# IN2-ViAUn/Exploration-of-Potential

Measured on AMD Instinct MI355X. Metric: training images/sec, YOLOX-l 24p 640x640 bf16, higher is better.
Workload: dtype bf16; 1 GPU; YOLOX-l-24p (CSPDarknet53+PAFPN+24p head) train step, 640x640, batch 20/GPU, 10 GTs/img, SimOTA + 24-circle GIoU loss, SGD nesterov; global_batch=20, parallelism=dp1, hip_graph=forward and backward as two lanes of captured segments, loss, update

## Files before the change

### exploration-of-potential_amd/csrc/elementwise.hip

```cpp
#include <stdio.h>
#include <stdlib.h>
#include "common.h"

namespace {

constexpr int MAX_BLOCKS = 2048;

__device__ __forceinline__ void load8(const bf16* p, float (&v)[8]) {
    bf16x8 t = *reinterpret_cast<const bf16x8*>(p);
#pragma unroll
    for (int i = 0; i < 8; ++i) v[i] = (float)t[i];
}
__device__ __forceinline__ void store8(bf16* p, const float (&v)[8]) {
    bf16x8 t;
#pragma unroll
    for (int i = 0; i < 8; ++i) t[i] = (bf16)v[i];
    *reinterpret_cast<bf16x8*>(p) = t;
}

struct RowMap {
    int tpr, rpb;
    __device__ RowMap(int C, int nt = 256) { tpr = C >> 3; rpb = tpr >= nt ? 1 : nt / tpr; }
};

template <int ACT, bool RES>
__global__ __launch_bounds__(256) void bn_act_fwd_kernel(const bf16* z, long ld_z, const long long* stats, int reps,
                                                         const float* gamma, const float* beta, float* rmean,
                                                         float* rvar, long* nbt, long* nbt2, float* save, bf16* y, long ld_y,
                                                         const bf16* res_, long ld_res, long M, int C, float eps,
                                                         float momentum) {
    constexpr int act = ACT;
    const bf16* res = RES ? res_ : nullptr;
    extern __shared__ float lds[];
    const int CP = C + (C >> 3);
    float* sc = lds;
    float* sh = lds + CP;
    auto pad = [](int c) { return c + (c >> 3); };
    for (int c = threadIdx.x; c < C; c += 256) {
        long long i1 = 0, i2 = 0;
        const float gmm = gamma[c], bta = beta[c];
        for (int rb = 0; rb < reps; rb += 8) {
            long long a[8], b[8];
#pragma unroll
            for (int r = 0; r < 8; ++r) {
                const int rr = rb + r < reps ? rb + r : rb;
                a[r] = stats[(long)rr * 2 * C + c];
                b[r] = stats[(long)rr * 2 * C + C + c];
            }
#pragma unroll
            for (int r = 0; r < 8; ++r) {
                i1 += rb + r < reps ? a[r] : 0ll;
                i2 += rb + r < reps ? b[r] : 0ll;
            }
        }
        const float mean = from_fix(i1) / (float)M;
        float var = from_fix(i2) / (float)M - mean * mean;
        var = var < 0.f ? 0.f : var;
        const float invstd = rsqrtf(var + eps);
        const float s_ = gmm * invstd;
        sc[pad(c)] = s_;
        sh[pad(c)] = bta - mean * s_;
        if (blockIdx.x == 0) {
            save[c] = mean;
            save[C + c] = invstd;
            if (rmean) {
                const float unb = M > 1 ? var * (float)M / (float)(M - 1) : var;
                rmean[c] = (1.f - momentum) * rmean[c] + momentum * mean;
                rvar[c] = (1.f - momentum) * rvar[c] + momentum * unb;
            }
        }
    }
    if (blockIdx.x == 0 && threadIdx.x == 0) {
        if (nbt) *nbt += 1;
        if (nbt2) *nbt2 += 1;
    }
    __syncthreads();
    const int cgs = C >> 3;
    const long total = M * cgs;
    const long stride = (long)gridDim.x * 256;
    constexpr int U = 4;
    const bool fixed_group = stride % cgs == 0;
    const int g_fixed = (int)(((long)blockIdx.x * 256 + threadIdx.x) % cgs);
    float rsc[8], rsh[8];
#pragma unroll
    for (int j = 0; j < 8; ++j) { rsc[j] = sc[g_fixed * 9 + j]; rsh[j] = sh[g_fixed * 9 + j]; }
    const long m_fixed = ((long)blockIdx.x * 256 + threadIdx.x) / cgs, m_step = stride / cgs;
    int it = 0;
    for (long i = (long)blockIdx.x * 256 + threadIdx.x; i < total; i += U * stride, ++it) {
        long mm[U];
        int gg[U];
        bf16x8 v[U], r[U];
#pragma unroll
        for (int k = 0; k < U; ++k) {
            const long ik = i + k * stride;
            const bool ok = ik < total;
            if (fixed_group) {
                mm[k] = ok ? m_fixed + (long)(it * U + k) * m_step : -1;
                gg[k] = g_fixed;
            } else {
                mm[k] = ok ? ik / cgs : -1;
                gg[k] = ok ? (int)(ik - mm[k] * cgs) : 0;
            }
            if (ok) {
                v[k] = *reinterpret_cast<const bf16x8*>(z + mm[k] * ld_z + gg[k] * 8);
                if constexpr (RES) r[k] = *reinterpret_cast<const bf16x8*>(res + mm[k] * ld_res + gg[k] * 8);
            }
        }
#pragma unroll
        for (int k = 0; k < U; ++k) {
            if (mm[k] < 0) break;
            bf16x8 o;
#pragma unroll
            for (int j = 0; j < 8; ++j) {
                const float a_ = fixed_group ? rsc[j] : sc[gg[k] * 9 + j];
                const float b_ = fixed_group ? rsh[j] : sh[gg[k] * 9 + j];
                const float u = fmaf((float)v[k][j], a_, b_);
                if constexpr (RES) o[j] = (bf16)(act_fwd(u, act) + (float)r[k][j]);
                else o[j] = (bf16)act_fwd(u, act);
            }
            *reinterpret_cast<bf16x8*>(y + mm[k] * ld_y + gg[k] * 8) = o;
        }
    }
}


template <int UNROLL, int NT, int ACT>
__device__ __forceinline__ void bn_bwd_reduce_body(const bf16* dy, long ld_dy, const bf16* z, long ld_z,
                                                   const float* save, const float* gamma,
                                                   const float* beta, long long* dgamma, long long* dbeta,
                                                   long M, int C, int reps, const int bid, const int nblk) {
    constexpr int act = ACT;
    __shared__ float red[NT][8 + 1];
    const RowMap rm(C, NT);
    const int tid = threadIdx.x;
    for (int cg0 = 0; cg0 < (C >> 3); cg0 += NT) {
        const int cg = cg0 + tid % rm.tpr;
        const int slot = rm.tpr >= NT ? 0 : tid / rm.tpr;
        const bool active = slot < rm.rpb && cg < (C >> 3);
        float sg[8] = {0, 0, 0, 0, 0, 0, 0, 0}, sb[8] = {0, 0, 0, 0, 0, 0, 0, 0};
        if (active) {
            const long step = (long)nblk * rm.rpb;
            const long m_first = (long)bid * rm.rpb + slot;
            bf16x8 vdy[UNROLL], vz[UNROLL];
#pragma unroll
            for (int k = 0; k < UNROLL; ++k) {
                const long mm = m_first + k * step < M ? m_first + k * step : (m_first < M ? m_first : 0);
                vdy[k] = *reinterpret_cast<const bf16x8*>(dy + mm * ld_dy + cg * 8);
                vz[k] = *reinterpret_cast<const bf16x8*>(z + mm * ld_z + cg * 8);
            }
            __builtin_amdgcn_sched_barrier(0);
            float sc[8], sh[8], iv[8], mi[8];
#pragma unroll
            for (int j = 0; j < 8; ++j) {
                const int c = cg * 8 + j;
                const float mean = save[c], inv = save[C + c];
                sc[j] = gamma[c] * inv; sh[j] = beta[c] - mean * sc[j]; iv[j] = inv; mi[j] = mean * inv;
            }
            for (long m = m_first; m < M; m += UNROLL * step) {
#pragma unroll
                for (int k = 0; k < UNROLL; ++k) {
                    if (m + k * step >= M) break;
#pragma unroll
                    for (int j = 0; j < 8; ++j) {
                        const float zz = (float)vz[k][j];
                        const float du = (float)vdy[k][j] * act_grad(fmaf(zz, sc[j], sh[j]), act);
                        sb[j] += du;
                        sg[j] = fmaf(du, fmaf(zz, iv[j], -mi[j]), sg[j]);
                    }
                }
                if (m + UNROLL * step < M) {
#pragma unroll
                    for (int k = 0; k < UNROLL; ++k) {
                        const long mn = m + (UNROLL + k) * step;
                        const long mm = mn < M ? mn : m;
                        vdy[k] = *reinterpret_cast<const bf16x8*>(dy + mm * ld_dy + cg * 8);
                        vz[k] = *reinterpret_cast<const bf16x8*>(z + mm * ld_z + cg * 8);
                    }
                }
            }
        }
        const int ngrp = min(min(rm.tpr, NT), (C >> 3) - cg0);
#pragma unroll
        for (int half = 0; half < 2; ++half) {
#pragma unroll
            for (int j = 0; j < 8; ++j) red[tid][j] = half ? sb[j] : sg[j];
            __syncthreads();
            for (int t = tid; t < ngrp * 8; t += NT) {
                const int g = t >> 3, v = t & 7;
                float a = 0.f;
                for (int sl = 0; sl < rm.rpb; ++sl) a += red[sl * rm.tpr + g][v];
                long long* dst = (half ? dbeta : dgamma) + (long)(bid % reps) * 2 * C + (cg0 + g) * 8 + v;
                atomicAdd((unsigned long long*)dst, (unsigned long long)to_fix_g(a));
            }
            __syncthreads();
        }
    }
}

template <int UNROLL, int NT, int ACT>
__global__ __launch_bounds__(NT) void bn_act_bwd_reduce_kernel(const bf16* dy, long ld_dy, const bf16* z, long ld_z,
                                                               const float* save, const float* gamma,
                                                               const float* beta, long long* dgamma, long long* dbeta,
                                                               long M, int C, int reps) {
    bn_bwd_reduce_body<UNROLL, NT, ACT>(dy, ld_dy, z, ld_z, save, gamma, beta, dgamma, dbeta, M, C, reps, (int)blockIdx.x, (int)gridDim.x);
}

template <int UNROLL, int ACT, bool ACC, bool COH>
__device__ __forceinline__ void bn_bwd_apply_body(const bf16* dy, long ld_dy, const bf16* z, long ld_z,
                                                  const float* save, const float* gamma, const float* beta,
                                                  const long long* dgamma, const long long* dbeta, float* ggrad,
                                                  float* bgrad, bf16* dz, long ld_dz, long M, int C, int reps, const int bid, const int nblk) {
    constexpr int act = ACT;
    const RowMap rm(C);
    const int tid = threadIdx.x;
    const float invM = 1.f / (float)M;
    extern __shared__ float folded[];
    for (int i = tid; i < 2 * C; i += 256) {
        const long long* src = i < C ? dgamma + i : dbeta + (i - C);
        long long acc = 0;
        bool bad = false;
        for (int rb = 0; rb < reps; rb += 8) {
            long long a[8];
#pragma unroll
            for (int r = 0; r < 8; ++r) {
                const long long* q = src + (long)(rb + r < reps ? rb + r : rb) * 2 * C;
                a[r] = COH ? __hip_atomic_load(q, __ATOMIC_RELAXED, __HIP_MEMORY_SCOPE_AGENT) : *q;
            }
#pragma unroll
            for (int r = 0; r < 8; ++r) {
                acc += rb + r < reps ? a[r] : 0ll;
                bad = bad || fixg_bad(a[r]);
            }
        }
        folded[i] = bad ? __builtin_nanf("") : from_fix_g(acc);
    }
    __syncthreads();
    for (int cg = tid % rm.tpr; cg < (C >> 3); cg += 256) {
        const int slot = rm.tpr >= 256 ? 0 : tid / rm.tpr;
        if (slot >= rm.rpb) break;
        float sc[8], sh[8], k1[8], k2[8], k3[8];
        float cm[8], ci[8], cg_[8], cb[8], csg[8], csb[8];
        {
            const f32x4* pm = reinterpret_cast<const f32x4*>(save + cg * 8);
            const f32x4* pi = reinterpret_cast<const f32x4*>(save + C + cg * 8);
            const f32x4* pg = reinterpret_cast<const f32x4*>(gamma + cg * 8);
            const f32x4* pb = reinterpret_cast<const f32x4*>(beta + cg * 8);
            const f32x4 m0 = pm[0], m1 = pm[1], i0 = pi[0], i1 = pi[1], g0 = pg[0], g1 = pg[1], b0 = pb[0], b1 = pb[1];
            const f32x4 s0 = *reinterpret_cast<const f32x4*>(folded + cg * 8), s1 = *reinterpret_cast<const f32x4*>(folded + cg * 8 + 4);
            const f32x4 t0 = *reinterpret_cast<const f32x4*>(folded + C + cg * 8), t1 = *reinterpret_cast<const f32x4*>(folded + C + cg * 8 + 4);
#pragma unroll
            for (int j = 0; j < 4; ++j) {
                cm[j] = m0[j]; cm[4 + j] = m1[j]; ci[j] = i0[j]; ci[4 + j] = i1[j]; cg_[j] = g0[j]; cg_[4 + j] = g1[j]; cb[j] = b0[j]; cb[4 + j] = b1[j];
                csg[j] = s0[j]; csg[4 + j] = s1[j]; csb[j] = t0[j]; csb[4 + j] = t1[j];
            }
        }
#pragma unroll
        for (int j = 0; j < 8; ++j) {
            const float mean = cm[j], inv = ci[j], g = cg_[j];
            const float sg_ = csg[j], sb_ = csb[j];
            sc[j] = g * inv; sh[j] = cb[j] - mean * sc[j];
            k1[j] = g * inv;
            k3[j] = k1[j] * inv * (sg_ * invM);
            k2[j] = k1[j] * (sb_ * invM) - k3[j] * mean;
        }
        if (bid == 0 && slot == 0 && ggrad) {
            f32x4* pgg = reinterpret_cast<f32x4*>(ggrad + cg * 8);
            f32x4* pbg = reinterpret_cast<f32x4*>(bgrad + cg * 8);
            f32x4 a0 = pgg[0], a1 = pgg[1], c0 = pbg[0], c1 = pbg[1];
#pragma unroll
            for (int j = 0; j < 4; ++j) {
                a0[j] += csg[j]; a1[j] += csg[4 + j];
                c0[j] += csb[j]; c1[j] += csb[4 + j];
            }
            pgg[0] = a0; pgg[1] = a1; pbg[0] = c0; pbg[1] = c1;
        }
        const long step = (long)nblk * rm.rpb;
        for (long m = (long)bid * rm.rpb + slot; m < M; m += UNROLL * step) {
            bf16x8 vdy[UNROLL], vz[UNROLL];
#pragma unroll
            for (int k = 0; k < UNROLL; ++k) {
                const long mm = m + k * step;
                if (mm < M) {
                    vdy[k] = __builtin_nontemporal_load(reinterpret_cast<const bf16x8*>(dy + mm * ld_dy + cg * 8));
                    vz[k] = __builtin_nontemporal_load(reinterpret_cast<const bf16x8*>(z + mm * ld_z + cg * 8));
                }
            }
#pragma unroll
            for (int k = 0; k < UNROLL; ++k) {
                const long mm = m + k * step;
                if (mm >= M) break;
                bf16x8 o;
#pragma unroll
                for (int j = 0; j < 8; ++j) {
                    const float zz = (float)vz[k][j];
                    const float du = (float)vdy[k][j] * act_grad(fmaf(zz, sc[j], sh[j]), act);
                    o[j] = (bf16)fmaf(-k3[j], zz, fmaf(k1[j], du, -k2[j]));
                }
                if (ACC) {
                    const bf16x8 old = *reinterpret_cast<const bf16x8*>(dz + mm * ld_dz + cg * 8);
#pragma unroll
                    for (int j = 0; j < 8; ++j) o[j] = (bf16)((float)old[j] + (float)o[j]);
                }
                *reinterpret_cast<bf16x8*>(dz + mm * ld_dz + cg * 8) = o;
            }
        }
    }
}

template <int UNROLL, int ACT, bool ACC = false>
__global__ __launch_bounds__(256) void bn_act_bwd_apply_kernel(const bf16* dy, long ld_dy, const bf16* z, long ld_z,
                                                               const float* save, const float* gamma, const float* beta,
                                                               const long long* dgamma, const long long* dbeta, float* ggrad,
                                                               float* bgrad, bf16* dz, long ld_dz, long M, int C, int reps) {
    bn_bwd_apply_body<UNROLL, ACT, ACC, false>(dy, ld_dy, z, ld_z, save, gamma, beta, dgamma, dbeta, ggrad, bgrad, dz, ld_dz, M, C, reps,
                                               (int)blockIdx.x, (int)gridDim.x);
}

__device__ unsigned g_bn_barrier_timeouts;

template <int ACT>
__global__ __launch_bounds__(256) void bn_act_bwd_fused_kernel(const bf16* dy, long ld_dy, const bf16* z, long ld_z,
                                                               const float* save, const float* gamma, const float* beta,
                                                               long long* dgamma, long long* dbeta, float* ggrad, float* bgrad,
                                                               bf16* dz, long ld_dz, long M, int C, int reps, unsigned* bar) {
    const int bid = (int)blockIdx.x, nblk = (int)gridDim.x;
    bn_bwd_reduce_body<4, 256, ACT>(dy, ld_dy, z, ld_z, save, gamma, beta, dgamma, dbeta, M, C, reps, bid, nblk);
    __syncthreads();
    if (threadIdx.x == 0) {
        __threadfence();
        __hip_atomic_fetch_add(bar, 1u, __ATOMIC_RELEASE, __HIP_MEMORY_SCOPE_AGENT);
        int tries = 0;
        while (__hip_atomic_load(bar, __ATOMIC_ACQUIRE, __HIP_MEMORY_SCOPE_AGENT) < (unsigned)nblk) {
            __builtin_amdgcn_s_sleep(2);
            if (++tries > (1 << 16)) { atomicAdd(&g_bn_barrier_timeouts, 1u); break; }
        }
    }
    __syncthreads();
    bn_bwd_apply_body<4, ACT, false, true>(dy, ld_dy, z, ld_z, save, gamma, beta, dgamma, dbeta, ggrad, bgrad, dz, ld_dz, M, C, reps, bid, nblk);
}

int flat_grid(long M, int C, int per_thread) {
    long blocks = (M * (C >> 3) + 256L * per_thread - 1) / (256L * per_thread);
    return (int)(blocks < 1 ? 1 : (blocks > MAX_BLOCKS ? MAX_BLOCKS : blocks));
}
int rows_grid(long M, int C, int rows_per_thread, int max_blocks, int nt = 256) {
    int tpr = C >> 3;
    int rpb = tpr >= nt ? 1 : nt / tpr;
    long blocks = (M + (long)rpb * rows_per_thread - 1) / ((long)rpb * rows_per_thread);
    return (int)(blocks < 1 ? 1 : (blocks > max_blocks ? max_blocks : blocks));
}

__global__ __launch_bounds__(256) void stem_pack_kernel(const float* img, bf16* rows, int B, int IH, int IW, int ld) {
    constexpr int TP = 32;
    __shared__ __attribute__((aligned(16))) bf16 tile[TP][120];
    const int FH = IH >> 1, FW = IW >> 1;
    const long npix = (long)B * FH * FW;
    const int chunks = ld >> 3;
    for (long p0 = (long)blockIdx.x * TP; p0 < npix; p0 += (long)gridDim.x * TP) {
        for (int it = threadIdx.x; it < 9 * TP; it += 256) {
            const int tap = it / TP, lp = it - tap * TP;
            const long pix = p0 + lp;
            float v[12] = {0.f, 0.f, 0.f, 0.f, 0.f, 0.f, 0.f, 0.f, 0.f, 0.f, 0.f, 0.f};
            if (pix < npix) {
                const int n = (int)(pix / ((long)FH * FW));
                const int rem = (int)(pix - (long)n * FH * FW);
                const int oy = rem / FW, ox = rem - oy * FW;
                const int fy = oy + tap / 3 - 1, fx = ox + tap % 3 - 1;
                if (fy >= 0 && fy < FH && fx >= 0 && fx < FW) {
#pragma unroll
                    for (int ch = 0; ch < 3; ++ch)
#pragma unroll
                        for (int yp = 0; yp < 2; ++yp) {
                            const float2 t = *reinterpret_cast<const float2*>(img + (((long)n * 3 + ch) * IH + 2 * fy + yp) * IW + 2 * fx);
                            v[(0 * 2 + yp) * 3 + ch] = t.x;
                            v[(1 * 2 + yp) * 3 + ch] = t.y;
                        }
                }
            }
#pragma unroll
            for (int j = 0; j < 12; ++j) tile[lp][tap * 12 + j] = (bf16)v[j];
        }
        if (threadIdx.x < TP) {
#pragma unroll
            for (int j = 108; j < 120; ++j) tile[threadIdx.x][j] = (bf16)0.f;
        }
        __syncthreads();
        for (int it = threadIdx.x; it < TP * chunks; it += 256) {
            const int lp = it / chunks, c = it - lp * chunks;
            const long pix = p0 + lp;
            if (pix >= npix) continue;
            bf16x8 o = {0, 0, 0, 0, 0, 0, 0, 0};
            if (c * 8 < 120) o = *reinterpret_cast<const bf16x8*>(&tile[lp][c * 8]);
            *reinterpret_cast<bf16x8*>(rows + pix * ld + c * 8) = o;
        }
        __syncthreads();
    }
}

__global__ __launch_bounds__(256) void focus_pack_kernel(const float* img, bf16* out, int B, int IH, int IW) {
    const int FH = IH >> 1, FW = IW >> 1;
    const long npix = (long)B * FH * FW;
    for (long pix = (long)blockIdx.x * 256 + threadIdx.x; pix < npix; pix += (long)gridDim.x * 256) {
        const int n = (int)(pix / ((long)FH * FW));
        const int rem = (int)(pix - (long)n * FH * FW);
        const int fy = rem / FW, fx = rem - fy * FW;
        float v[12];
#pragma unroll
        for (int ch = 0; ch < 3; ++ch)
#pragma unroll
            for (int yp = 0; yp < 2; ++yp) {
                const float2 t = *reinterpret_cast<const float2*>(img + (((long)n * 3 + ch) * IH + 2 * fy + yp) * IW + 2 * fx);
                v[(0 * 2 + yp) * 3 + ch] = t.x;
                v[(1 * 2 + yp) * 3 + ch] = t.y;
            }
        bf16x8 lo, hi = {0, 0, 0, 0, 0, 0, 0, 0};
#pragma unroll
        for (int j = 0; j < 8; ++j) lo[j] = (bf16)v[j];
#pragma unroll
        for (int j = 8; j < 12; ++j) hi[j - 8] = (bf16)v[j];
        *reinterpret_cast<bf16x8*>(out + pix * 16) = lo;
        *reinterpret_cast<bf16x8*>(out + pix * 16 + 8) = hi;
    }
}

__global__ __launch_bounds__(256) void spp_fwd_kernel(const bf16* x, long ld_x, bf16* y5, bf16* y9, bf16* y13, long ld_y,
                                                      uint8_t* idx, int B, int H, int W, int C) {
    const int cgs = C >> 3;
    const long total = (long)B * H * W * cgs;
    const long plane = (long)B * H * W * C;
    for (long i = (long)blockIdx.x * 256 + threadIdx.x; i < total; i += (long)gridDim.x * 256) {
        const int cg = (int)(i % cgs);
        const long pix = i / cgs;
        const int n = (int)(pix / (H * W));
        const int rem = (int)(pix - (long)n * H * W);
        const int py = rem / W, px = rem - py * W;
        float m5[8], m9[8], m13[8];
        uint8_t i5[8], i9[8], i13[8];
#pragma unroll
        for (int j = 0; j < 8; ++j) { m5[j] = m9[j] = m13[j] = -INFINITY; i5[j] = i9[j] = i13[j] = 0x88; }
        for (int dy = -6; dy <= 6; ++dy) {
            const int yy = py + dy;
            if (yy < 0 || yy >= H) continue;
            for (int dx = -6; dx <= 6; ++dx) {
                const int xx = px + dx;
                if (xx < 0 || xx >= W) continue;
                float v[8];
                load8(x + ((long)(n * H + yy) * W + xx) * ld_x + cg * 8, v);
                const uint8_t code = (uint8_t)(((dy + 8) << 4) | (dx + 8));
                const bool in9 = dy >= -4 && dy <= 4 && dx >= -4 && dx <= 4;
                const bool in5 = dy >= -2 && dy <= 2 && dx >= -2 && dx <= 2;
#pragma unroll
                for (int j = 0; j < 8; ++j) {
                    if (v[j] > m13[j] || v[j] != v[j]) { m13[j] = v[j]; i13[j] = code; }
                    if (in9 && (v[j] > m9[j] || v[j] != v[j])) { m9[j] = v[j]; i9[j] = code; }
                    if (in5 && (v[j] > m5[j] || v[j] != v[j])) { m5[j] = v[j]; i5[j] = code; }
                }
            }
        }
        store8(y5 + pix * ld_y + cg * 8, m5);
        store8(y9 + pix * ld_y + cg * 8, m9);
        store8(y13 + pix * ld_y + cg * 8, m13);
        uint8_t* ip = idx + pix * C + cg * 8;
#pragma unroll
        for (int j = 0; j < 8; ++j) { ip[j] = i5[j]; ip[plane + j] = i9[j]; ip[2 * plane + j] = i13[j]; }
    }
}

__global__ __launch_bounds__(256) void spp_row_kernel(const bf16* x, long ld_x, bf16* h, uint8_t* hx, int B, int H, int W, int C) {
    const int cgs = C >> 3;
    const long total = (long)B * H * W * cgs;
    const long plane = (long)B * H * W * C;
    for (long i = (long)blockIdx.x * 256 + threadIdx.x; i < total; i += (long)gridDim.x * 256) {
        const int cg = (int)(i % cgs);
        const long pix = i / cgs;
        const int px = (int)(pix % W);
        float m5[8], m9[8], m13[8];
        uint8_t i5[8], i9[8], i13[8];
#pragma unroll
        for (int j = 0; j < 8; ++j) { m5[j] = m9[j] = m13[j] = -INFINITY; i5[j] = i9[j] = i13[j] = 8; }
#pragma unroll
        for (int dx = -6; dx <= 6; ++dx) {
            const int xx = px + dx;
            if (xx < 0 || xx >= W) continue;
            float v[8];
            load8(x + (pix + dx) * ld_x + cg * 8, v);
            const uint8_t code = (uint8_t)(dx + 8);
            const bool in9 = dx >= -4 && dx <= 4, in5 = dx >= -2 && dx <= 2;
#pragma unroll
            for (int j = 0; j < 8; ++j) {
                if (v[j] > m13[j] || v[j] != v[j]) { m13[j] = v[j]; i13[j] = code; }
                if (in9 && (v[j] > m9[j] || v[j] != v[j])) { m9[j] = v[j]; i9[j] = code; }
                if (in5 && (v[j] > m5[j] || v[j] != v[j])) { m5[j] = v[j]; i5[j] = code; }
            }
        }
        bf16* hp = h + pix * C + cg * 8;
        store8(hp, m5); store8(hp + plane, m9); store8(hp + 2 * plane, m13);
        uint8_t* ip = hx + pix * C + cg * 8;
#pragma unroll
        for (int j = 0; j < 8; ++j) { ip[j] = i5[j]; ip[plane + j] = i9[j]; ip[2 * plane + j] = i13[j]; }
    }
}

__global__ __launch_bounds__(256) void spp_col_kernel(const bf16* h, const uint8_t* hx, bf16* y5, bf16* y9, bf16* y13, long ld_y,
                                                      uint8_t* idx, int B, int H, int W, int C) {
    const int cgs = C >> 3;
    const long total = (long)B * H * W * cgs;
    const long plane = (long)B * H * W * C;
    for (long i = (long)blockIdx.x * 256 + threadIdx.x; i < total; i += (long)gridDim.x * 256) {
        const int cg = (int)(i % cgs);
        const long pix = i / cgs;
        const int py = (int)((pix / W) % H);
        float m[3][8];
        uint8_t id[3][8];
#pragma unroll
        for (int w = 0; w < 3; ++w)
#pragma unroll
            for (int j = 0; j < 8; ++j) { m[w][j] = -INFINITY; id[w][j] = 0x88; }
#pragma unroll
        for (int dy = -6; dy <= 6; ++dy) {
            const int yy = py + dy;
            if (yy < 0 || yy >= H) continue;
            const long q = (pix + (long)dy * W) * C + cg * 8;
#pragma unroll
            for (int w = 0; w < 3; ++w) {
                const int r = 2 + 2 * w;
                if (dy < -r || dy > r) continue;
                float v[8];
                load8(h + w * plane + q, v);
                const uint2 cx = *reinterpret_cast<const uint2*>(hx + w * plane + q);
#pragma unroll
                for (int j = 0; j < 8; ++j) {
                    const unsigned c = ((j < 4 ? cx.x : cx.y) >> (8 * (j & 3))) & 0xFF;
                    if (v[j] > m[w][j] || v[j] != v[j]) { m[w][j] = v[j]; id[w][j] = (uint8_t)(((dy + 8) << 4) | c); }
                }
            }
        }
        store8(y5 + pix * ld_y + cg * 8, m[0]);
        store8(y9 + pix * ld_y + cg * 8, m[1]);
        store8(y13 + pix * ld_y + cg * 8, m[2]);
        uint8_t* ip = idx + pix * C + cg * 8;
#pragma unroll
        for (int j = 0; j < 8; ++j) { ip[j] = id[0][j]; ip[plane + j] = id[1][j]; ip[2 * plane + j] = id[2][j]; }
    }
}

__global__ __launch_bounds__(256) void spp_bwd_kernel(const bf16* dy5, const bf16* dy9, const bf16* dy13, long ld_dy,
                                                      const uint8_t* idx, bf16* dx, long ld_dx, int accumulate, int B,
                                                      int H, int W, int C) {
    const int cgs = C >> 3;
    const long total = (long)B * H * W * cgs;
    const long plane = (long)B * H * W * C;
    for (long i = (long)blockIdx.x * 256 + threadIdx.x; i < total; i += (long)gridDim.x * 256) {
        const int cg = (int)(i % cgs);
        const long pix = i / cgs;
        const int n = (int)(pix / (H * W));
        const int rem = (int)(pix - (long)n * H * W);
        const int py = rem / W, px = rem - py * W;
        float acc[8] = {0, 0, 0, 0, 0, 0, 0, 0};
        for (int dy = -6; dy <= 6; ++dy) {
            const int oy = py - dy;
            if (oy < 0 || oy >= H) continue;
            for (int dxo = -6; dxo <= 6; ++dxo) {
                const int ox = px - dxo;
                if (ox < 0 || ox >= W) continue;
                const long op = (long)(n * H + oy) * W + ox;
                const uint8_t code = (uint8_t)(((dy + 8) << 4) | (dxo + 8));
                const uint8_t* ip = idx + op * C + cg * 8;
                const unsigned rep = code * 0x01010101u;
                auto gather = [&](const bf16* g, const uint8_t* codes) {
                    uint2 c = *reinterpret_cast<const uint2*>(codes);
                    c.x ^= rep; c.y ^= rep;
                    float v[8];
                    load8(g + op * ld_dy + cg * 8, v);
#pragma unroll
                    for (int j = 0; j < 8; ++j)
                        if ((((j < 4 ? c.x : c.y) >> (8 * (j & 3))) & 0xFFu) == 0u) acc[j] += v[j];
                };
                gather(dy13, ip + 2 * plane);
                if (dy >= -4 && dy <= 4 && dxo >= -4 && dxo <= 4) gather(dy9, ip + plane);
                if (dy >= -2 && dy <= 2 && dxo >= -2 && dxo <= 2) gather(dy5, ip);
            }
        }
        bf16* d = dx + pix * ld_dx + cg * 8;
        if (accumulate) {
            float o[8];
            load8(d, o);
#pragma unroll
            for (int j = 0; j < 8; ++j) acc[j] += o[j];
        }
        store8(d, acc);
    }
}

__global__ __launch_bounds__(256) void spp_bwd_lds_kernel(const bf16* dy5, const bf16* dy9, const bf16* dy13, long ld_dy,
                                                          const uint8_t* idx, bf16* dx, long ld_dx, int accumulate, int B,
                                                          int H, int W, int C) {
    extern __shared__ __attribute__((aligned(16))) char spp_lds[];
    const int HW = H * W;
    bf16x8* gv = reinterpret_cast<bf16x8*>(spp_lds);
    uint2* cv = reinterpret_cast<uint2*>(spp_lds + (size_t)3 * HW * 16);
    float* gh = reinterpret_cast<float*>(spp_lds + (size_t)3 * HW * 24);
    uint2* ds = reinterpret_cast<uint2*>(spp_lds + (size_t)3 * HW * 24 + (size_t)HW * 32);
    const int cg = blockIdx.x, n = blockIdx.y;
    const long plane = (long)B * HW * C;
    const long base = (long)n * HW;
    for (int q = threadIdx.x; q < HW; q += 256) {
        const long op = base + q;
        gv[q] = *reinterpret_cast<const bf16x8*>(dy5 + op * ld_dy + cg * 8);
// ... 816 lines not shown
```

Measured before the change: 1037 images/s.

## Prefetch BN activation tiles before stat reduction and software-pipeline elementwise loops

In the BN+activation forward and the backward apply kernels, the first batch of replica statistics, per-channel constants and the first U rows of activations are now loaded before the per-channel stat fold and the __syncthreads. Sched barriers keep the compiler from sinking those loads. The main loops are rotated so that the next iteration's rows are loaded while the current rows are computed and stored, with a separate tail epilogue. The aim is to hide global-load latency behind the reduction and compute phases. In exchange it uses more registers, which may reduce occupancy, and it issues clamped loads at safe indices for out-of-range rows.

```diff
diff --git a/exploration-of-potential_amd/csrc/elementwise.hip b/exploration-of-potential_amd/csrc/elementwise.hip
--- a/exploration-of-potential_amd/csrc/elementwise.hip
+++ b/exploration-of-potential_amd/csrc/elementwise.hip
@@ -36,23 +36,23 @@
     float* sc = lds;
     float* sh = lds + CP;
     auto pad = [](int c) { return c + (c >> 3); };
-    for (int c = threadIdx.x; c < C; c += 256) {
-        long long i1 = 0, i2 = 0;
-        const float gmm = gamma[c], bta = beta[c];
-        for (int rb = 0; rb < reps; rb += 8) {
-            long long a[8], b[8];
-#pragma unroll
-            for (int r = 0; r < 8; ++r) {
-                const int rr = rb + r < reps ? rb + r : rb;
-                a[r] = stats[(long)rr * 2 * C + c];
-                b[r] = stats[(long)rr * 2 * C + C + c];
-            }
-#pragma unroll
-            for (int r = 0; r < 8; ++r) {
-                i1 += rb + r < reps ? a[r] : 0ll;
-                i2 += rb + r < reps ? b[r] : 0ll;
-            }
-        }
+    const int tid = threadIdx.x;
+    auto load_batch = [&](int c, int rb, long long (&a)[8], long long (&b)[8]) {
+#pragma unroll
+        for (int r = 0; r < 8; ++r) {
+            const int rr = rb + r < reps ? rb + r : rb;
+            a[r] = stats[(long)rr * 2 * C + c];
+            b[r] = stats[(long)rr * 2 * C + C + c];
+        }
+    };
+    auto add_batch = [&](int rb, const long long (&a)[8], const long long (&b)[8], long long& i1, long long& i2) {
+#pragma unroll
+        for (int r = 0; r < 8; ++r) {
+            i1 += rb + r < reps ? a[r] : 0ll;
+            i2 += rb + r < reps ? b[r] : 0ll;
+        }
+    };
+    auto finish = [&](int c, long long i1, long long i2, float gmm, float bta) {
         const float mean = from_fix(i1) / (float)M;
         float var = from_fix(i2) / (float)M - mean * mean;
         var = var < 0.f ? 0.f : var;
@@ -69,57 +69,115 @@
                 rvar[c] = (1.f - momentum) * rvar[c] + momentum * unb;
             }
         }
-    }
-    if (blockIdx.x == 0 && threadIdx.x == 0) {
-        if (nbt) *nbt += 1;
-        if (nbt2) *nbt2 += 1;
-    }
-    __syncthreads();
+    };
+    const int c_first = tid < C ? tid : 0;
+    long long a0[8], b0[8];
+    load_batch(c_first, 0, a0, b0);
+    const float g0 = gamma[c_first], bt0 = beta[c_first];
+    __builtin_amdgcn_sched_barrier(0);
+
     const int cgs = C >> 3;
     const long total = M * cgs;
     const long stride = (long)gridDim.x * 256;
     constexpr int U = 4;
-    const bool fixed_group = stride % cgs == 0;
-    const int g_fixed = (int)(((long)blockIdx.x * 256 + threadIdx.x) % cgs);
+    const unsigned i_first = blockIdx.x * 256u + (unsigned)tid, ustride = gridDim.x * 256u;
+    const bool fixed_group = ustride % (unsigned)cgs == 0;
+    const int g_fixed = (int)(i_first % (unsigned)cgs);
+    const long m_fixed = (long)(i_first / (unsigned)cgs), m_step = (long)(ustride / (unsigned)cgs);
+    const bool any = (long)i_first < total;
+    const long m_safe = any ? m_fixed : 0;
+    const int g_safe = any ? g_fixed : 0;
+    struct Where { long m; int g; };
+    auto locate = [&](long ik, int n) __attribute__((always_inline)) {
+        const bool ok = ik < total;
+        Where w;
+        if (fixed_group) {
+            w.m = ok ? m_fixed + (long)n * m_step : m_safe;
+            w.g = g_safe;
+        } else {
+            w.m = ok ? ik / cgs : m_safe;
+            w.g = ok ? (int)(ik - w.m * cgs) : g_safe;
+        }
+        return w;
+    };
+    long mm[U];
+    int gg[U];
+    bf16x8 v[U], r[U];
+#pragma unroll
+    for (int k = 0; k < U; ++k) {
+        const Where w = locate((long)i_first + k * stride, k);
+        mm[k] = w.m; gg[k] = w.g;
+    }
+#pragma unroll
+    for (int k = 0; k < U; ++k) {
+        v[k] = *reinterpret_cast<const bf16x8*>(z + mm[k] * ld_z + gg[k] * 8);
+        if constexpr (RES) r[k] = *reinterpret_cast<const bf16x8*>(res + mm[k] * ld_res + gg[k] * 8);
+    }
+    __builtin_amdgcn_sched_barrier(0);
+
+    if (tid < C) {
+        long long i1 = 0, i2 = 0;
+        add_batch(0, a0, b0, i1, i2);
+        for (int rb = 8; rb < reps; rb += 8) {
+            long long a[8], b[8];
+            load_batch(tid, rb, a, b);
+            add_batch(rb, a, b, i1, i2);
+        }
+        finish(tid, i1, i2, g0, bt0);
+    }
+    for (int c = tid + 256; c < C; c += 256) {
+        long long i1 = 0, i2 = 0;
+        const float gmm = gamma[c], bta = beta[c];
+        for (int rb = 0; rb < reps; rb += 8) {
+            long long a[8], b[8];
+            load_batch(c, rb, a, b);
+            add_batch(rb, a, b, i1, i2);
+        }
+        finish(c, i1, i2, gmm, bta);
+    }
+    if (blockIdx.x == 0 && tid == 0) {
+        if (nbt) *nbt += 1;
+        if (nbt2) *nbt2 += 1;
+    }
+    __syncthreads();
     float rsc[8], rsh[8];
 #pragma unroll
     for (int j = 0; j < 8; ++j) { rsc[j] = sc[g_fixed * 9 + j]; rsh[j] = sh[g_fixed * 9 + j]; }
-    const long m_fixed = ((long)blockIdx.x * 256 + threadIdx.x) / cgs, m_step = stride / cgs;
+    auto compute = [&](int k) __attribute__((always_inline)) {
+        bf16x8 o;
+        float ca[8], cb[8];
+#pragma unroll
+        for (int j = 0; j < 8; ++j) { ca[j] = rsc[j]; cb[j] = rsh[j]; }
+        if (!fixed_group) {
+#pragma unroll
+            for (int j = 0; j < 8; ++j) { ca[j] = sc[gg[k] * 9 + j]; cb[j] = sh[gg[k] * 9 + j]; }
+        }
+#pragma unroll
+        for (int j = 0; j < 8; ++j) {
+            const float u = fmaf((float)v[k][j], ca[j], cb[j]);
+            if constexpr (RES) o[j] = (bf16)(act_fwd(u, act) + (float)r[k][j]);
+            else o[j] = (bf16)act_fwd(u, act);
+        }
+        return o;
+    };
+    long i = (long)i_first;
     int it = 0;
-    for (long i = (long)blockIdx.x * 256 + threadIdx.x; i < total; i += U * stride, ++it) {
-        long mm[U];
-        int gg[U];
-        bf16x8 v[U], r[U];
+    for (; i + U * stride < total; i += U * stride, ++it) {
 #pragma unroll
         for (int k = 0; k < U; ++k) {
-            const long ik = i + k * stride;
-            const bool ok = ik < total;
-            if (fixed_group) {
-                mm[k] = ok ? m_fixed + (long)(it * U + k) * m_step : -1;
-                gg[k] = g_fixed;
-            } else {
-                mm[k] = ok ? ik / cgs : -1;
-                gg[k] = ok ? (int)(ik - mm[k] * cgs) : 0;
-            }
-            if (ok) {
-                v[k] = *reinterpret_cast<const bf16x8*>(z + mm[k] * ld_z + gg[k] * 8);
-                if constexpr (RES) r[k] = *reinterpret_cast<const bf16x8*>(res + mm[k] * ld_res + gg[k] * 8);
-            }
-        }
-#pragma unroll
-        for (int k = 0; k < U; ++k) {
-            if (mm[k] < 0) break;
-            bf16x8 o;
-#pragma unroll
-            for (int j = 0; j < 8; ++j) {
-                const float a_ = fixed_group ? rsc[j] : sc[gg[k] * 9 + j];
-                const float b_ = fixed_group ? rsh[j] : sh[gg[k] * 9 + j];
-                const float u = fmaf((float)v[k][j], a_, b_);
-                if constexpr (RES) o[j] = (bf16)(act_fwd(u, act) + (float)r[k][j]);
-                else o[j] = (bf16)act_fwd(u, act);
-            }
-            *reinterpret_cast<bf16x8*>(y + mm[k] * ld_y + gg[k] * 8) = o;
-        }
+            const bf16x8 o = compute(k);
+            bf16* dst = y + mm[k] * ld_y + gg[k] * 8;
+            const Where w = locate(i + (U + k) * stride, (it + 1) * U + k);
+            mm[k] = w.m; gg[k] = w.g;
+            v[k] = *reinterpret_cast<const bf16x8*>(z + mm[k] * ld_z + gg[k] * 8);
+            if constexpr (RES) r[k] = *reinterpret_cast<const bf16x8*>(res + mm[k] * ld_res + gg[k] * 8);
+            *reinterpret_cast<bf16x8*>(dst) = o;
+        }
+    }
+#pragma unroll
+    for (int k = 0; k < U; ++k) {
+        if (i + k * stride >= total) break;
+        *reinterpret_cast<bf16x8*>(y + mm[k] * ld_y + gg[k] * 8) = compute(k);
     }
 }
 
@@ -215,37 +273,78 @@
     const int tid = threadIdx.x;
     const float invM = 1.f / (float)M;
     extern __shared__ float folded[];
-    for (int i = tid; i < 2 * C; i += 256) {
+    auto load_replicas = [&](int i, int rb, long long (&a)[8]) {
         const long long* src = i < C ? dgamma + i : dbeta + (i - C);
+#pragma unroll
+        for (int r = 0; r < 8; ++r) {
+            const long long* q = src + (long)(rb + r < reps ? rb + r : rb) * 2 * C;
+            a[r] = COH ? __hip_atomic_load(q, __ATOMIC_RELAXED, __HIP_MEMORY_SCOPE_AGENT) : *q;
+        }
+    };
+    auto add_replicas = [&](int rb, const long long (&a)[8], long long& acc, bool& bad) {
+#pragma unroll
+        for (int r = 0; r < 8; ++r) {
+            acc += rb + r < reps ? a[r] : 0ll;
+            bad = bad || fixg_bad(a[r]);
+        }
+    };
+    f32x4 m0, m1, i0, i1, g0, g1, b0, b1;
+    auto load_consts = [&](int cg) {
+        const f32x4* pm = reinterpret_cast<const f32x4*>(save + cg * 8);
+        const f32x4* pi = reinterpret_cast<const f32x4*>(save + C + cg * 8);
+        const f32x4* pg = reinterpret_cast<const f32x4*>(gamma + cg * 8);
+        const f32x4* pb = reinterpret_cast<const f32x4*>(beta + cg * 8);
+        m0 = pm[0]; m1 = pm[1]; i0 = pi[0]; i1 = pi[1]; g0 = pg[0]; g1 = pg[1]; b0 = pb[0]; b1 = pb[1];
+    };
+    const int slot = rm.tpr >= 256 ? 0 : tid / rm.tpr;
+    const long step = (long)nblk * rm.rpb;
+    const long m_first = (long)bid * rm.rpb + slot;
+    const long m_safe = m_first < M ? m_first : 0;
+    bf16x8 vdy[UNROLL], vz[UNROLL];
+    auto load_row = [&](int k, long mm, int cg) {
+        vdy[k] = __builtin_nontemporal_load(reinterpret_cast<const bf16x8*>(dy + mm * ld_dy + cg * 8));
+        vz[k] = __builtin_nontemporal_load(reinterpret_cast<const bf16x8*>(z + mm * ld_z + cg * 8));
+    };
+    auto load_first_rows = [&](int cg) {
+#pragma unroll
+        for (int k = 0; k < UNROLL; ++k) load_row(k, m_first + k * step < M ? m_first + k * step : m_safe, cg);
+    };
+
+    const int e_first = tid < 2 * C ? tid : 0;
+    long long a0[8];
+    load_replicas(e_first, 0, a0);
+    int cg = tid % rm.tpr;
+    load_consts(cg);
+    load_first_rows(cg);
+    __builtin_amdgcn_sched_barrier(0);
+
+    if (tid < 2 * C) {
+        long long acc = 0;
+        bool bad = false;
+        add_replicas(0, a0, acc, bad);
+        for (int rb = 8; rb < reps; rb += 8) {
+            long long a[8];
+            load_replicas(tid, rb, a);
+            add_replicas(rb, a, acc, bad);
+        }
+        folded[tid] = bad ? __builtin_nanf("") : from_fix_g(acc);
+    }
+    for (int i = tid + 256; i < 2 * C; i += 256) {
         long long acc = 0;
         bool bad = false;
         for (int rb = 0; rb < reps; rb += 8) {
             long long a[8];
-#pragma unroll
-            for (int r = 0; r < 8; ++r) {
-                const long long* q = src + (long)(rb + r < reps ? rb + r : rb) * 2 * C;
-                a[r] = COH ? __hip_atomic_load(q, __ATOMIC_RELAXED, __HIP_MEMORY_SCOPE_AGENT) : *q;
-            }
-#pragma unroll
-            for (int r = 0; r < 8; ++r) {
-                acc += rb + r < reps ? a[r] : 0ll;
-                bad = bad || fixg_bad(a[r]);
-            }
+            load_replicas(i, rb, a);
+            add_replicas(rb, a, acc, bad);
         }
         folded[i] = bad ? __builtin_nanf("") : from_fix_g(acc);
     }
     __syncthreads();
-    for (int cg = tid % rm.tpr; cg < (C >> 3); cg += 256) {
-        const int slot = rm.tpr >= 256 ? 0 : tid / rm.tpr;
-        if (slot >= rm.rpb) break;
+    if (slot >= rm.rpb) return;
+    for (;;) {
         float sc[8], sh[8], k1[8], k2[8], k3[8];
         float cm[8], ci[8], cg_[8], cb[8], csg[8], csb[8];
         {
-            const f32x4* pm = reinterpret_cast<const f32x4*>(save + cg * 8);
-            const f32x4* pi = reinterpret_cast<const f32x4*>(save + C + cg * 8);
-            const f32x4* pg = reinterpret_cast<const f32x4*>(gamma + cg * 8);
-            const f32x4* pb = reinterpret_cast<const f32x4*>(beta + cg * 8);
-            const f32x4 m0 = pm[0], m1 = pm[1], i0 = pi[0], i1 = pi[1], g0 = pg[0], g1 = pg[1], b0 = pb[0], b1 = pb[1];
             const f32x4 s0 = *reinterpret_cast<const f32x4*>(folded + cg * 8), s1 = *reinterpret_cast<const f32x4*>(folded + cg * 8 + 4);
             const f32x4 t0 = *reinterpret_cast<const f32x4*>(folded + C + cg * 8), t1 = *reinterpret_cast<const f32x4*>(folded + C + cg * 8 + 4);
 #pragma unroll
@@ -266,44 +365,51 @@
         if (bid == 0 && slot == 0 && ggrad) {
             f32x4* pgg = reinterpret_cast<f32x4*>(ggrad + cg * 8);
             f32x4* pbg = reinterpret_cast<f32x4*>(bgrad + cg * 8);
-            f32x4 a0 = pgg[0], a1 = pgg[1], c0 = pbg[0], c1 = pbg[1];
+            f32x4 a0_ = pgg[0], a1_ = pgg[1], c0_ = pbg[0], c1_ = pbg[1];
 #pragma unroll
             for (int j = 0; j < 4; ++j) {
-                a0[j] += csg[j]; a1[j] += csg[4 + j];
-                c0[j] += csb[j]; c1[j] += csb[4 + j];
-            }
-            pgg[0] = a0; pgg[1] = a1; pbg[0] = c0; pbg[1] = c1;
-        }
-        const long step = (long)nblk * rm.rpb;
-        for (long m = (long)bid * rm.rpb + slot; m < M; m += UNROLL * step) {
-            bf16x8 vdy[UNROLL], vz[UNROLL];
+                a0_[j] += csg[j]; a1_[j] += csg[4 + j];
+                c0_[j] += csb[j]; c1_[j] += csb[4 + j];
+            }
+            pgg[0] = a0_; pgg[1] = a1_; pbg[0] = c0_; pbg[1] = c1_;
+        }
+        auto row = [&](int k, long mm) {
+            bf16x8 o;
+#pragma unroll
+            for (int j = 0; j < 8; ++j) {
+                const float zz = (float)vz[k][j];
+                const float du = (float)vdy[k][j] * act_grad(fmaf(zz, sc[j], sh[j]), act);
+                o[j] = (bf16)fmaf(-k3[j], zz, fmaf(k1[j], du, -k2[j]));
+            }
+            return o;
+        };
+        auto put = [&](bf16x8 o, long mm) {
+            if (ACC) {
+                const bf16x8 old = *reinterpret_cast<const bf16x8*>(dz + mm * ld_dz + cg * 8);
+#pragma unroll
+                for (int j = 0; j < 8; ++j) o[j] = (bf16)((float)old[j] + (float)o[j]);
+            }
+            *reinterpret_cast<bf16x8*>(dz + mm * ld_dz + cg * 8) = o;
+        };
+        long m = m_first;
+        for (; m + UNROLL * step < M; m += UNROLL * step) {
 #pragma unroll
             for (int k = 0; k < UNROLL; ++k) {
-                const long mm = m + k * step;
-                if (mm < M) {
-                    vdy[k] = __builtin_nontemporal_load(reinterpret_cast<const bf16x8*>(dy + mm * ld_dy + cg * 8));
-                    vz[k] = __builtin_nontemporal_load(reinterpret_cast<const bf16x8*>(z + mm * ld_z + cg * 8));
-                }
-            }
-#pragma unroll
-            for (int k = 0; k < UNROLL; ++k) {
-                const long mm = m + k * step;
-                if (mm >= M) break;
-                bf16x8 o;
-#pragma unroll
-                for (int j = 0; j < 8; ++j) {
-                    const float zz = (float)vz[k][j];
-                    const float du = (float)vdy[k][j] * act_grad(fmaf(zz, sc[j], sh[j]), act);
-                    o[j] = (bf16)fmaf(-k3[j], zz, fmaf(k1[j], du, -k2[j]));
-                }
-                if (ACC) {
-                    const bf16x8 old = *reinterpret_cast<const bf16x8*>(dz + mm * ld_dz + cg * 8);
-#pragma unroll
-                    for (int j = 0; j < 8; ++j) o[j] = (bf16)((float)old[j] + (float)o[j]);
-                }
-                *reinterpret_cast<bf16x8*>(dz + mm * ld_dz + cg * 8) = o;
-            }
-        }
+                const bf16x8 o = row(k, m + k * step);
+                const long mn = m + (UNROLL + k) * step;
+                load_row(k, mn < M ? mn : m, cg);
+                put(o, m + k * step);
+            }
+        }
+#pragma unroll
+        for (int k = 0; k < UNROLL; ++k) {
+            if (m + k * step >= M) break;
+            put(row(k, m + k * step), m + k * step);
+        }
+        cg += 256;
+        if (cg >= (C >> 3)) break;
+        load_consts(cg);
+        load_first_rows(cg);
     }
 }
 
```

After: 1045 images/s, median of 6. No clear change (+0.8%).
